# VinAIResearch/Counting-DETR

Hardware: AMD Instinct MI355X
Metric: images/sec FSCD-147 2nd-stage train step (higher is better)
Workload: dtype forward bf16x3 (fp32 operands split hi+lo, 3 bf16 MFMAs per product); data / weight gradients bf16 (both operands rounded to bf16, 1 MFMA per product); fp32 accumulate, fp32 storage, fp32 attention softmax / norms / losses / optimizer; 1 GPU; FSCD-147 2nd-stage train step (ResNet-50-DC5 + RCDA enc6/dec6, Q=300 learned, 800x800, T=[37, 120]), fwd+matcher+loss+bwd+clip+AdamW; images_per_gpu=2, global_batch=2, parallelism=dp1, graph=True, precision=bf16x3, precision_backward=bf16, frozen_stage_prefetch=True

## Files before the change

### counting_detr_amd/csrc/api.hip

```cpp
#include <stdarg.h>
#include <stdio.h>

#include "../../include/cdetr_hip.h"
#include "common.h"

static thread_local char g_err[512] = "";

void cdetr_set_error(const char* fmt, ...) {
    va_list ap;
    va_start(ap, fmt);
    vsnprintf(g_err, sizeof(g_err), fmt, ap);
    va_end(ap);
}

extern "C" const char* cdetr_last_error(void) { return g_err; }
extern "C" int cdetr_abi_version(void) { return CDETR_ABI_VERSION; }

#include <stdlib.h>
#include <string.h>
extern char** environ;
namespace {
struct TuneEnvCheck {
    TuneEnvCheck() {
        if (getenv("CDETR_TUNING") != nullptr || environ == nullptr) return;
        static const char* const knobs[] = {"CDETR_DIRECT_MAX_BLOCKS", "CDETR_GEMM_DL", "CDETR_GEMM_FEWROW_SPLIT", "CDETR_GEMM_SPLITK", "CDETR_GEMM_VARIANT",
                                            "CDETR_LN_BWD_ROWS", "CDETR_LSAP_GENERIC", "CDETR_RCDA_HS", "CDETR_RCDA_PROBE", "CDETR_WGRAD_KP",
                                            "CDETR_WGRAD_VARIANT"};
        for (const char* k : knobs)
            if (getenv(k) != nullptr)
                fprintf(stderr, "libcdetr_hip: %s is set but CDETR_TUNING is not -- per-call tuning knobs are ignored without it\n", k);
    }
} g_tune_env_check;
}
```

### counting_detr_amd/csrc/rcda.hip

```cpp
#include "../../include/cdetr_hip.h"
#include "common.h"
#include <algorithm>
#include <type_traits>
#include <stdlib.h>

namespace {

__device__ __forceinline__ void xcd_slab(int& bx, int& by) {
    const int gx = gridDim.x, total = gx * gridDim.y;
    if (total & 7) return;
    const int lin = by * gx + bx;
    const int l2 = (lin & 7) * (total >> 3) + (lin >> 3);
    by = l2 / gx;
    bx = l2 - by * gx;
}


constexpr int D = 32;
constexpr int QW = 32;

__device__ __forceinline__ float4 ld4(const float* p) { return *reinterpret_cast<const float4*>(p); }

struct FwdSmem {
    int sw, sh;
// ... 204 lines not shown
                                 : make_float4(0.f, 0.f, 0.f, 0.f);

    const float* vbase = d.v + (long)n * H * W * E + head * D;
    constexpr int VSLOTS = (NF * 256 + NT - 1) / NT;
    float4 rv[VSLOTS];
    auto vfetch = [&](int w) {
#pragma unroll
        for (int s = 0; s < VSLOTS; ++s) {
            const int idx = tid + NT * s;
            const int h = idx >> 3, c4 = idx & 7;
            rv[s] = (h < H) ? ld4(vbase + ((long)h * W + w) * E + c4 * 4) : make_float4(0.f, 0.f, 0.f, 0.f);
        }
    };
    auto vstash = [&](int buf) {
#pragma unroll
        for (int s = 0; s < VSLOTS; ++s) {
            const int idx = tid + NT * s;
            const int h = idx >> 3, c4 = idx & 7;
            if (h < H) *reinterpret_cast<float4*>(Vs + buf * Hp * D + h * D + c4 * 4) = rv[s];
        }
    };
    f32x16 acc;
#pragma unroll
    for (int r = 0; r < 16; ++r) acc[r] = 0.f;
    vfetch(0);
    vstash(0);
    __syncthreads();
    for (int w = 0; w < W; ++w) {
        const int buf = w & 1;
        if (w + 1 < W) vfetch(w + 1);
        const float arow = Srow[i32 * sm.sw + w];
        const float* vb = Vs + buf * Hp * D + (g * 4) * D + i32;
        if (PREC == 0) {
#pragma unroll
            for (int kk = 0; kk < KH8; ++kk) {
                if (kk * 8 < Hp) {
                    const float p0 = acol[kk].x * arow, p1 = acol[kk].y * arow, p2 = acol[kk].z * arow, p3 = acol[kk].w * arow;
                    const float b0 = vb[(kk * 8 + 0) * D], b1 = vb[(kk * 8 + 1) * D], b2 = vb[(kk * 8 + 2) * D],
                                b3 = vb[(kk * 8 + 3) * D];
                    acc = __builtin_amdgcn_mfma_f32_32x32x2f32(p0, b0, acc, 0, 0, 0);
                    acc = __builtin_amdgcn_mfma_f32_32x32x2f32(p1, b1, acc, 0, 0, 0);
                    acc = __builtin_amdgcn_mfma_f32_32x32x2f32(p2, b2, acc, 0, 0, 0);
                    acc = __builtin_amdgcn_mfma_f32_32x32x2f32(p3, b3, acc, 0, 0, 0);
                }
            }
        } else {
#pragma unroll
            for (int kp = 0; kp < KH8 / 2; ++kp) {
                if (kp * 16 < Hp) {
                    const int k0 = 2 * kp, k1 = 2 * kp + 1;
                    const bool has1 = k1 * 8 < Hp;
                    const float pa[8] = {acol[k0].x * arow, acol[k0].y * arow, acol[k0].z * arow, acol[k0].w * arow,
                                         acol[k1].x * arow, acol[k1].y * arow, acol[k1].z * arow, acol[k1].w * arow};
                    float vv[8];
#pragma unroll
                    for (int t = 0; t < 4; ++t) {
                        vv[t] = vb[(k0 * 8 + t) * D];
                        vv[4 + t] = has1 ? vb[(k1 * 8 + t) * D] : 0.f;
                    }
                    bf16x8 ah, al, bh, bl;
                    split_bf16x8(pa, ah, al);
                    split_bf16x8(vv, bh, bl);
                    acc = mfma_bf16x3(ah, al, bh, bl, acc);
                }
            }
        }
        if (w + 1 < W) vstash(buf ^ 1);
        __syncthreads();
    }
    mfma_drain(acc);
#pragma unroll
    for (int r = 0; r < 16; ++r) {
        const int qq = qbase + (r & 3) + 8 * (r >> 2) + 4 * g;
        if (qq < L) d.out[((long)n * L + qq) * E + head * D + i32] = acc[r];
    }
}

constexpr int RCDA_WS_COUNTERS = 4096;
constexpr int KSTR = 36;

template <int NT, int TW, int TH, bool PROBE = false>
__device__ __forceinline__ void rcda_scores_mfma(const cdetr_rcda_fwd_desc& d, const FwdSmem& sm, float* smem, float* Srow, float* Scol,
                                                 int tid, int lane, int i32, int g, int n, int head, int qbase, int q, bool qvalid,
                                                 bool save = true, unsigned long long* stamps = nullptr) {
    auto stamp = [&](int i) __attribute__((always_inline)) {
        if constexpr (PROBE) { stamps[i] = __builtin_amdgcn_s_memtime(); asm volatile("s_waitcnt lgkmcnt(0)" ::: "memory"); }
    };
    const int H = d.H, W = d.W, L = d.L, E = d.nh * D;
    const int Wp = (W + 3) & ~3, Hp = (H + 7) & ~7;
    float* Krow = smem + sm.off_k;
    float* Kcol = Krow + W * KSTR;
    {
        const int nk8 = (W + H) * 8;
        for (int base = 0; base < nk8; base += 4 * NT) {
            float4 t[4];
#pragma unroll
            for (int u = 0; u < 4; ++u) {
                const int idx = min(base + tid + NT * u, nk8 - 1);
                const int key = idx >> 3, c4 = idx & 7;
                const float* src = (key < W) ? d.k_row + ((long)n * W + key) * E + head * D + c4 * 4
                                             : d.k_col + ((long)n * H + (key - W)) * E + head * D + c4 * 4;
                t[u] = ld4(src);
            }
#pragma unroll
            for (int u = 0; u < 4; ++u) {
                const int idx = base + tid + NT * u;
                if (idx < nk8) *reinterpret_cast<float4*>(Krow + (idx >> 3) * KSTR + (idx & 7) * 4) = t[u];
            }
        }
    }
    bf16x8 qh[2][2], ql[2][2];
#pragma unroll
    for (int side = 0; side < 2; ++side) {
        const float* qp = (side == 0 ? d.q_row : d.q_col) + ((long)n * L + (qvalid ? q : 0)) * E + head * D + 8 * g;
#pragma unroll
        for (int st = 0; st < 2; ++st) {
            float4 t0 = ld4(qp + 16 * st), t1 = ld4(qp + 16 * st + 4);
            if (!qvalid) { t0 = make_float4(0.f, 0.f, 0.f, 0.f); t1 = t0; }
            const float x[8] = {t0.x, t0.y, t0.z, t0.w, t1.x, t1.y, t1.z, t1.w};
            split_bf16x8(x, qh[side][st], ql[side][st]);
        }
    }
    unsigned long long mrow[2] = {0ull, 0ull}, mcol[2] = {0ull, 0ull};
    if (d.mask_row) {
        const uint8_t* mr = d.mask_row + (long)n * W;
        const uint8_t* mc = d.mask_col + (long)n * H;
        mrow[0] = __ballot(lane < W && mr[min(lane, W - 1)] != 0);
        mcol[0] = __ballot(lane < H && mc[min(lane, H - 1)] != 0);
        if (TW > 2) mrow[1] = __ballot(lane + 64 < W && mr[min(lane + 64, W - 1)] != 0);
        if (TH > 2) mcol[1] = __ballot(lane + 64 < H && mc[min(lane + 64, H - 1)] != 0);
    }
    if constexpr (PROBE) { asm volatile("s_waitcnt vmcnt(0)" ::: "memory"); }
    stamp(0);
    __syncthreads();
    stamp(1);

#pragma unroll
    for (int side = 0; side < 2; ++side) {
        constexpr int TMAX = TW > TH ? TW : TH;
        const int nt = side == 0 ? TW : TH;
        const int nkeys = side == 0 ? W : H, npad = side == 0 ? Wp : Hp;
        const float* Ks = side == 0 ? Krow : Kcol;
        const unsigned long long* mbits = side == 0 ? mrow : mcol;
        float* S = side == 0 ? Srow + i32 * sm.sw : Scol + i32 * sm.sh;
        float sv[TMAX][16];
        float mx = -INFINITY;
#pragma unroll
        for (int t = 0; t < TMAX; ++t) {
            if (t >= nt) break;
            const int kc = min(32 * t + i32, nkeys - 1);
            f32x16 acc = {0.f, 0.f, 0.f, 0.f, 0.f, 0.f, 0.f, 0.f, 0.f, 0.f, 0.f, 0.f, 0.f, 0.f, 0.f, 0.f};
#pragma unroll
            for (int st = 0; st < 2; ++st) {
                const float4 t0 = *reinterpret_cast<const float4*>(Ks + kc * KSTR + 16 * st + 8 * g);
                const float4 t1 = *reinterpret_cast<const float4*>(Ks + kc * KSTR + 16 * st + 8 * g + 4);
                const float x[8] = {t0.x, t0.y, t0.z, t0.w, t1.x, t1.y, t1.z, t1.w};
                bf16x8 ah, al;
                split_bf16x8(x, ah, al);
                acc = mfma_bf16x3(ah, al, qh[side][st], ql[side][st], acc);
            }
            mfma_drain(acc);
            const unsigned chunk = (unsigned)(mbits[t >> 1] >> (32 * (t & 1)));
            const int lim = nkeys - 32 * t - 4 * g;
            const unsigned dead = (chunk >> (4 * g)) | (lim >= 32 ? 0u : (lim <= 0 ? 0xffffffffu : (0xffffffffu << lim)));
#pragma unroll
            for (int r = 0; r < 16; ++r) {
                constexpr unsigned one = 1u;
                const unsigned bit = one << ((r & 3) + 8 * (r >> 2));
                const float v = (dead & bit) ? -INFINITY : acc[r] * d.scale;
                sv[t][r] = v;
                mx = fmaxf(mx, v);
            }
        }
        mx = xhalf_max(mx);
        float sum = 0.f;
#pragma unroll
        for (int t = 0; t < TMAX; ++t) {
            if (t >= nt) break;
#pragma unroll
            for (int r = 0; r < 16; ++r) {
                const float e = __expf(sv[t][r] - mx);
                sv[t][r] = e;
                sum += e;
            }
        }
        sum = xhalf_sum(sum);
        const float inv = 1.f / sum;
#pragma unroll
        for (int t = 0; t < TMAX; ++t) {
            if (t >= nt) break;
#pragma unroll
            for (int r = 0; r < 16; ++r) {
                const int key = 32 * t + (r & 3) + 8 * (r >> 2) + 4 * g;
                S[min(key, npad)] = sv[t][r] * inv;
            }
        }
        stamp(2 + side);
    }
    __syncthreads();
    stamp(4);

    {
        const int nq = min(QW, L - qbase);
        if (nq > 0 && save && d.a_row != nullptr) {
            save_rows(Srow, sm.sw, d.a_row + (((long)n * d.nh + head) * L + qbase) * Wp, nq, Wp, lane);
            save_rows(Scol, sm.sh, d.a_col + (((long)n * d.nh + head) * L + qbase) * Hp, nq, Hp, lane);
        }
    }
    stamp(5);
}

struct Fwd2Smem { int off_v, vts, total; };
__host__ __device__ inline Fwd2Smem fwd2_smem(const FwdSmem& sm, int H, int W, int KS) {
    Fwd2Smem s;
    s.off_v = sm.off_k;
    s.vts = 32 * KS + 8;
    const int vfloats = 2 * 32 * s.vts / 2;
    const int kfloats = (W + H) * KSTR;
    s.total = sm.off_k + (kfloats > vfloats ? kfloats : vfloats);
    return s;
}

template <int NW, int KS, int TH = 2, bool PROBE = false>
__global__ __launch_bounds__(64 * NW) void rcda_fwd2_kernel(const cdetr_rcda_fwd_desc d) {
    unsigned long long pt[5] = {0, 0, 0, 0, 0}, pacc[3] = {0, 0, 0};
    auto now = [&]() __attribute__((always_inline)) -> unsigned long long {
        if constexpr (PROBE) { const unsigned long long t = __builtin_amdgcn_s_memtime(); asm volatile("s_waitcnt lgkmcnt(0)" ::: "memory"); return t; }
        return 0ull;
    };
    pt[0] = now();
    constexpr int NT = 64 * NW, QB = QW * NW;
    constexpr int PD = 4;
    constexpr int NBLK = 16 * 4 * KS;
    constexpr int VB = (NBLK + NT - 1) / NT;
    constexpr int VTS = 32 * KS + 8;
    extern __shared__ __attribute__((aligned(16))) float smem[];
    const int H = d.H, W = d.W, L = d.L, E = d.nh * D;
    const FwdSmem sm = fwd_smem(H, W, NW);
    const int tid = threadIdx.x, lane = tid & 63, wid = tid >> 6;
    const int i32 = lane & 31, g = lane >> 5;
    int bx_ = blockIdx.x, by_ = blockIdx.y;
    xcd_slab(bx_, by_);
    const int n = by_ / d.nh, head = by_ % d.nh;
    const int qbase = bx_ * QB + wid * QW;
    const int q = qbase + i32;
    const bool qvalid = q < L;
    float* Srow = smem + sm.off_srow + wid * QW * sm.sw;
    float* Scol = smem + sm.off_scol + wid * QW * sm.sh;
    const int hs = gridDim.z, hz = blockIdx.z;
    const int hper = (H + hs - 1) / hs;
    const int hb = hz * hper, he = min(H, hb + hper);
    __bf16* VT = reinterpret_cast<__bf16*>(smem + sm.off_k);
    const float* vsrc[VB];
    long vrow[VB][4];
    int vdst[VB];
#pragma unroll
    for (int b = 0; b < VB; ++b) {
        const int blk = tid + NT * b;
        const int wg = (blk < NBLK) ? (blk >> 4) : 0, cp = blk & 15;
        vdst[b] = (blk < NBLK) ? (2 * cp) * VTS + 4 * wg : -1;
        vsrc[b] = d.v + ((long)n * H + min(hb, H - 1)) * W * E + head * D + 2 * cp;
#pragma unroll
        for (int kk = 0; kk < 4; ++kk) vrow[b][kk] = (long)min(4 * wg + kk, W - 1) * E;
    }
    float rv[PD][VB][8];
    const long tileE = (long)W * E;
    int hf = min(hb, H - 1);
    auto vfetch = [&](float (&r)[VB][8]) __attribute__((always_inline)) {
#pragma unroll
        for (int b = 0; b < VB; ++b) {
#pragma unroll
            for (int kk = 0; kk < 4; ++kk) {
                const float2 t = *reinterpret_cast<const float2*>(vsrc[b] + vrow[b][kk]);
                r[b][2 * kk] = t.x;
                r[b][2 * kk + 1] = t.y;
            }
        }
        ++hf;
        if (hf < H) {
#pragma unroll
            for (int b = 0; b < VB; ++b) vsrc[b] += tileE;
        }
    };
    auto vstash = [&](const float (&r)[VB][8], int buf) __attribute__((always_inline)) {
#pragma unroll
        for (int b = 0; b < VB; ++b) {
            if (vdst[b] < 0) continue;
            __bf16* dst = VT + buf * 32 * VTS + vdst[b];
            stash_split4(dst, 16 * KS, r[b][0], r[b][2], r[b][4], r[b][6]);
            stash_split4(dst + VTS, 16 * KS, r[b][1], r[b][3], r[b][5], r[b][7]);
        }
    };

    unsigned long long sst[6] = {0, 0, 0, 0, 0, 0};
    if (H <= 32 * TH) rcda_scores_mfma<NT, (KS + 1) / 2, TH, PROBE>(d, sm, smem, Srow, Scol, tid, lane, i32, g, n, head, qbase, q, qvalid, hz == 0, sst);
    else rcda_scores<NT>(d, sm, smem, Srow, Scol, tid, lane, i32, g, n, head, qbase, q, qvalid);
    pt[1] = now();

    bf16x8 bh[KS], bl[KS];
#pragma unroll
    for (int s = 0; s < KS; ++s) {
        float x[8];
#pragma unroll
        for (int j = 0; j < 8; ++j) {
            const int w = 16 * s + 8 * g + j;
            x[j] = (w < W) ? Srow[i32 * sm.sw + w] : 0.f;
        }
        split_bf16x8(x, bh[s], bl[s]);
    }

    float outT[16];
#pragma unroll
    for (int r = 0; r < 16; ++r) outT[r] = 0.f;
    const f32x16 zero = {0.f, 0.f, 0.f, 0.f, 0.f, 0.f, 0.f, 0.f, 0.f, 0.f, 0.f, 0.f, 0.f, 0.f, 0.f, 0.f};

    vfetch(rv[0]); vfetch(rv[1]); vfetch(rv[2]); vfetch(rv[3]);
    vstash(rv[0], 0);
    __syncthreads();
    pt[2] = now();
    auto step = [&](auto U, int h) __attribute__((always_inline)) {
        constexpr int u = decltype(U)::value;
        const unsigned long long s0 = now();
        vfetch(rv[u]);
        const unsigned long long s1 = now();
        const float acolh = (h < he) ? Scol[i32 * sm.sh + h] : 0.f;
        const __bf16* vt = VT + (u & 1) * 32 * VTS + i32 * VTS + 8 * g;
        f32x16 T = zero;
#pragma unroll
        for (int s = 0; s < KS; ++s) {
            const bf16x8 ah = *reinterpret_cast<const bf16x8*>(vt + 16 * s);
            const bf16x8 al = *reinterpret_cast<const bf16x8*>(vt + 16 * KS + 16 * s);
            T = mfma_bf16x3(ah, al, bh[s], bl[s], T);
        }
#pragma unroll
        for (int r = 0; r < 16; ++r) outT[r] = fmaf(acolh, T[r], outT[r]);
        unsigned long long s2 = 0;
        if constexpr (PROBE) { asm volatile("" :: "v"(outT[0]), "v"(outT[15])); s2 = now(); }
        vstash(rv[(u + 1) % PD], (u + 1) & 1);
        const unsigned long long s3 = now();
        __syncthreads();
        if constexpr (PROBE) {
            const unsigned long long s4 = now();
            pacc[0] += s4 - s3; pacc[1] += s2 - s1; pacc[2] += (s1 - s0) + (s3 - s2);
        }
    };
    for (int h0 = hb; h0 < he; h0 += PD) {
        step(std::integral_constant<int, 0>{}, h0);
        step(std::integral_constant<int, 1>{}, h0 + 1);
        step(std::integral_constant<int, 2>{}, h0 + 2);
        step(std::integral_constant<int, 3>{}, h0 + 3);
    }
    pt[3] = now();
    if (hs > 1) {
        int* cnt = reinterpret_cast<int*>(d.ws);
        float* wsp = reinterpret_cast<float*>(cnt + RCDA_WS_COUNTERS);
        const int tile = blockIdx.y * gridDim.x + blockIdx.x;
        float* mine = wsp + ((long)tile * hs + hz) * 16 * NT + tid;
#pragma unroll
        for (int r = 0; r < 16; ++r) __hip_atomic_store(mine + r * NT, outT[r], __ATOMIC_RELAXED, __HIP_MEMORY_SCOPE_AGENT);
        __builtin_amdgcn_s_waitcnt(0);
        __syncthreads();
        int* flag = reinterpret_cast<int*>(smem + sm.off_k);
        if (tid == 0) {
            const int old = __hip_atomic_fetch_add(cnt + tile, 1, __ATOMIC_RELAXED, __HIP_MEMORY_SCOPE_AGENT);
            const int last = (old == hs - 1) ? 1 : 0;
            if (last) __hip_atomic_store(cnt + tile, 0, __ATOMIC_RELAXED, __HIP_MEMORY_SCOPE_AGENT);
            *flag = last;
        }
        __syncthreads();
        if (*flag == 0) return;
        float sum[16];
#pragma unroll
        for (int r = 0; r < 16; ++r) sum[r] = 0.f;
        for (int z = 0; z < hs; ++z) {
            if (z == hz) {
#pragma unroll
                for (int r = 0; r < 16; ++r) sum[r] += outT[r];
            } else {
                const float* other = wsp + ((long)tile * hs + z) * 16 * NT + tid;
                float t[16];
#pragma unroll
                for (int r = 0; r < 16; ++r) t[r] = __hip_atomic_load(other + r * NT, __ATOMIC_RELAXED, __HIP_MEMORY_SCOPE_AGENT);
#pragma unroll
                for (int r = 0; r < 16; ++r) sum[r] += t[r];
            }
        }
#pragma unroll
        for (int r = 0; r < 16; ++r) outT[r] = sum[r];
    }
    if (qvalid) {
        float* op = d.out + ((long)n * L + q) * E + head * D + 4 * g;
#pragma unroll
        for (int j = 0; j < 4; ++j)
            *reinterpret_cast<float4*>(op + 8 * j) = make_float4(outT[4 * j], outT[4 * j + 1], outT[4 * j + 2], outT[4 * j + 3]);
    }
    if constexpr (PROBE) {
        asm volatile("s_waitcnt vmcnt(0)" ::: "memory");
        pt[4] = now();
        if (lane == 0) {
            unsigned long long* o = reinterpret_cast<unsigned long long*>(d.ws) + ((long)(blockIdx.y * gridDim.x + blockIdx.x) * NW + wid) * 16;
            o[0] = pt[0]; o[1] = pt[1]; o[2] = pt[2]; o[3] = pt[3]; o[4] = pt[4]; o[5] = pacc[0]; o[6] = pacc[1]; o[7] = pacc[2];
#pragma unroll
            for (int i = 0; i < 6; ++i) o[8 + i] = sst[i];
        }
    }
}

constexpr int BWD_CG = 2;
struct BwdSmem {
    int sw, sh, su, off_u, off_r, off_kk, total;
};
__host__ __device__ inline BwdSmem bwd_smem(int H, int W, int NF, int NW, bool with_k = false) {
    BwdSmem s;
    const int Wp = (W + 3) & ~3, Hp = (H + 7) & ~7;
    s.sw = Wp + 1;
    s.sh = Hp + 1;
    s.su = s.sw > s.sh ? s.sw : s.sh;
    s.off_u = 0;
    int u = NW * QW * s.su;
    const int v = 2 * BWD_CG * (32 * NF) * 36;
    if (v > u) u = v;
    s.off_r = (u + 3) & ~3;
    s.total = s.off_r + NW * QW * s.sw;
    s.off_kk = (s.total + 3) & ~3;
    if (with_k) s.total = s.off_kk + (W + H) * D;
    return s;
}

template <int NF, int NW, int PREC, int TERMS = 3, bool PROBE = false>
__device__ __forceinline__ void rcda_bwd_body(const cdetr_rcda_bwd_desc& d, const int bx, const int by) {
    unsigned long long pst[7] = {0, 0, 0, 0, 0, 0, 0};
    auto stamp = [&](int i) __attribute__((always_inline)) {
        if constexpr (PROBE) { pst[i] = __builtin_amdgcn_s_memtime(); asm volatile("s_waitcnt lgkmcnt(0)" ::: "memory"); }
    };
    auto flush_probe = [&]() __attribute__((always_inline)) {
        if constexpr (PROBE) {
            asm volatile("s_waitcnt vmcnt(0)" ::: "memory");
            if ((threadIdx.x & 63) == 0) {
                unsigned long long* o = reinterpret_cast<unsigned long long*>(d.ds_row) + ((long)(by * gridDim.x + bx) * NW + (threadIdx.x >> 6)) * 16;
#pragma unroll
                for (int i = 0; i < 7; ++i) o[i] = pst[i];
            }
        }
    };
    stamp(0);
    constexpr int NT = 64 * NW, QB = QW * NW;
    extern __shared__ __attribute__((aligned(16))) float smem[];
    constexpr int VS = 36;
    constexpr int HR = 32 * NF;
    const int H = d.H, W = d.W, L = d.L, E = d.nh * D;
    const int Wp = (W + 3) & ~3, Hp = (H + 7) & ~7;
    const BwdSmem sm = bwd_smem(H, W, NF, NW, d.dq_row != nullptr);
    const int tid = threadIdx.x, lane = tid & 63, wid = tid >> 6;
    const int i32 = lane & 31, g = lane >> 5;
    const int n = by / d.nh, head = by % d.nh;
    const int qbase = bx * QB + wid * QW;
    const int q = qbase + i32;
    const bool qvalid = q < L;
    const int nq = min(QW, L - qbase);

    constexpr int KP = 4;
    const int nk8 = (W + H) * 8;
    const bool kpre_ok = d.dq_row != nullptr && nk8 <= KP * NT;
    float4 kpre[KP];
#pragma unroll
    for (int u = 0; u < KP; ++u) kpre[u] = make_float4(0.f, 0.f, 0.f, 0.f);
    if (kpre_ok) {
#pragma unroll
        for (int u = 0; u < KP; ++u) {
            const int idx = min(tid + NT * u, nk8 - 1);
            const int key = idx >> 3, c4 = idx & 7;
            const float* src = (key < W) ? d.k_row + ((long)n * W + key) * E + head * D + c4 * 4
                                         : d.k_col + ((long)n * H + (key - W)) * E + head * D + c4 * 4;
            kpre[u] = ld4(src);
        }
    }

    float* Acol = smem + sm.off_u + wid * QW * sm.su;
    float* Arow = smem + sm.off_r + wid * QW * sm.sw;
    float* dArow = Arow;
    float* Vs = smem + sm.off_u;

    float dob[4][4];
// ... 676 lines not shown
template <int NF, int NW>
int launch_rcda_bwd_all(const cdetr_rcda_bwd_desc& d, hipStream_t st, int hgroups, int slices, int per) {
    const int bytes = std::max(bwd_smem(d.H, d.W, NF, NW, d.dq_row != nullptr).total * 4, dv2_smem().total * 4);
    int rc;
    const int nqb = (d.L + QW * NW - 1) / (QW * NW);
    dim3 grid(nqb + hgroups * slices, d.N * d.nh);
    if (d.precision == 3) {
        if ((rc = set_smem(rcda_bwd_all_kernel<NF, NW, 1>, bytes, "cdetr_rcda_bwd"))) return rc;
        hipLaunchKernelGGL((rcda_bwd_all_kernel<NF, NW, 1>), grid, dim3(512), bytes, st, d, nqb, hgroups, per);
    } else {
        if ((rc = set_smem(rcda_bwd_all_kernel<NF, NW, 3>, bytes, "cdetr_rcda_bwd"))) return rc;
        hipLaunchKernelGGL((rcda_bwd_all_kernel<NF, NW, 3>), grid, dim3(512), bytes, st, d, nqb, hgroups, per);
    }
    return cdetr_launch_status("cdetr_rcda_bwd(dS+dV)");
}
template <int NF, int NW>
int launch_rcda_bwd(const cdetr_rcda_bwd_desc& d, hipStream_t st) {
    const BwdSmem sm = bwd_smem(d.H, d.W, NF, NW, d.dq_row != nullptr);
    const int bytes = sm.total * 4;
    int rc;
    dim3 grid((d.L + QW * NW - 1) / (QW * NW), d.N * d.nh), block(64 * NW);
    if constexpr (NF == 4) {
        if (d.precision == 3) {
            if ((rc = set_smem(rcda_bwd_kernel<NF, NW, 1, 1>, bytes, "cdetr_rcda_bwd"))) return rc;
            hipLaunchKernelGGL((rcda_bwd_kernel<NF, NW, 1, 1>), grid, block, bytes, st, d);
            return cdetr_launch_status("cdetr_rcda_bwd(dS)");
        }
        if (d.precision >= 1) {
            if ((rc = set_smem(rcda_bwd_kernel<NF, NW, 1>, bytes, "cdetr_rcda_bwd"))) return rc;
            hipLaunchKernelGGL((rcda_bwd_kernel<NF, NW, 1>), grid, block, bytes, st, d);
            return cdetr_launch_status("cdetr_rcda_bwd(dS)");
        }
    }
    if ((rc = set_smem(rcda_bwd_kernel<NF, NW, 0>, bytes, "cdetr_rcda_bwd"))) return rc;
    hipLaunchKernelGGL((rcda_bwd_kernel<NF, NW, 0>), grid, block, bytes, st, d);
    return cdetr_launch_status("cdetr_rcda_bwd(dS)");
}
inline bool rcda_wg5(int L, int NH) {
    const long wg4 = (long)((L + QW * 4 - 1) / (QW * 4)) * NH, wg5 = (long)((L + QW * 5 - 1) / (QW * 5)) * NH;
    return wg4 > 256 && wg4 <= 512 && wg5 <= 256;
}
inline int fwd2_slices(const cdetr_rcda_fwd_desc& d, int base, int nt, int lds_bytes) {
    if (!d.ws || base > RCDA_WS_COUNTERS) return 1;
    int hs;
    const char* f = cdetr_tune_env("CDETR_RCDA_HS");
    if (f) hs = atoi(f);
    else {
        const int per_cu = lds_bytes > 0 ? std::max(1, std::min(4, (160 * 1024) / lds_bytes)) : 1;
        (void)per_cu;
        hs = 256 / base;
    }
    hs = std::min(std::min(hs, 8), d.H / 8);
    const long avail = (long)d.ws_bytes - (long)RCDA_WS_COUNTERS * 4;
    while (hs > 1 && (long)base * hs * 16 * nt * 4 > avail) --hs;
    return hs < 1 ? 1 : hs;
}
inline int rcda_probe() {
    const char* p = cdetr_tune_env("CDETR_RCDA_PROBE");
    return p ? atoi(p) : 0;
}

}

extern "C" int cdetr_rcda_fwd(const cdetr_rcda_fwd_desc* dp, void* stream) {
    CDETR_CHECK_ARG(dp != nullptr, "cdetr_rcda_fwd: null descriptor");
    const cdetr_rcda_fwd_desc d = *dp;
    CDETR_CHECK_ARG(d.N > 0 && d.L > 0 && d.H > 0 && d.W > 0 && d.nh > 0, "cdetr_rcda_fwd: bad sizes");
    CDETR_CHECK_ARG(d.H <= 128 && d.W <= 1024, "cdetr_rcda_fwd: H must be <= 128 (got %d)", d.H);
    CDETR_CHECK_ARG(d.q_row && d.q_col && d.k_row && d.k_col && d.v && d.out, "cdetr_rcda_fwd: null pointer");
    CDETR_CHECK_ARG((d.a_row != nullptr) == (d.a_col != nullptr), "cdetr_rcda_fwd: a_row and a_col are saved together or not at all (both NULL: inference)");
    hipStream_t st = reinterpret_cast<hipStream_t>(stream);
    if (d.precision == 1 && d.W <= 96) {
        const int ks = (d.W + 15) / 16;
        auto go = [&](auto kern, int NWv, int KSv = 0, bool sliced = true) -> int {
            const FwdSmem sm = fwd_smem(d.H, d.W, NWv);
            const int bytes = fwd2_smem(sm, d.H, d.W, KSv ? KSv : ks).total * 4;
            int rc;
            if ((rc = set_smem(kern, bytes, "cdetr_rcda_fwd"))) return rc;
            dim3 grid((d.L + QW * NWv - 1) / (QW * NWv), d.N * d.nh), block(64 * NWv);
            if (sliced) grid.z = fwd2_slices(d, (int)(grid.x * grid.y), 64 * NWv, bytes);
            hipLaunchKernelGGL(kern, grid, block, bytes, st, d);
            return cdetr_launch_status("cdetr_rcda_fwd");
        };
        if (const int probe = rcda_probe(); probe && d.ws && ks == 4 && d.H <= 64)
            return probe == 5 ? go(rcda_fwd2_kernel<5, 4, 2, true>, 5, 0, false) : go(rcda_fwd2_kernel<4, 4, 2, true>, 4, 0, false);
        if (ks == 4 && rcda_wg5(d.L, d.N * d.nh)) return go(rcda_fwd2_kernel<5, 4>, 5);
        if (ks > 4 || d.H > 64) {
            if (d.H > 64 && d.H <= 96) return ks <= 4 ? go(rcda_fwd2_kernel<4, 4, 3>, 4, 4) : go(rcda_fwd2_kernel<4, 6, 3>, 4, 6);
            if (ks <= 4) return go(rcda_fwd2_kernel<4, 4>, 4, 4);
            return ks == 5 ? go(rcda_fwd2_kernel<4, 5>, 4) : go(rcda_fwd2_kernel<4, 6>, 4);
        }
        if (ks == 1) return go(rcda_fwd2_kernel<4, 1>, 4);
        if (ks == 2) return go(rcda_fwd2_kernel<4, 2>, 4);
        if (ks == 3) return go(rcda_fwd2_kernel<4, 3>, 4);
        return go(rcda_fwd2_kernel<4, 4>, 4);
    }
    if (d.H <= 32) return launch_rcda_fwd<1>(d, st);
    if (d.H <= 64) return launch_rcda_fwd<2>(d, st);
    return launch_rcda_fwd<4>(d, st);
}

extern "C" int cdetr_rcda_bwd(const cdetr_rcda_bwd_desc* dp, void* stream) {
    CDETR_CHECK_ARG(dp != nullptr, "cdetr_rcda_bwd: null descriptor");
    const cdetr_rcda_bwd_desc d = *dp;
    CDETR_CHECK_ARG(d.N > 0 && d.L > 0 && d.H > 0 && d.W > 0 && d.nh > 0, "cdetr_rcda_bwd: bad sizes");
    CDETR_CHECK_ARG(d.H <= 128 && d.W <= 1024, "cdetr_rcda_bwd: H must be <= 128 (got %d)", d.H);
    CDETR_CHECK_ARG(d.d_out && d.a_row && d.a_col && d.v && d.d_v, "cdetr_rcda_bwd: null pointer");
    CDETR_CHECK_ARG((d.ds_row && d.ds_col) || (!d.ds_row && !d.ds_col && d.dk_row),
                    "cdetr_rcda_bwd: ds_row / ds_col may only be omitted (both) when the fused q / k gradients are requested");
    CDETR_CHECK_ARG(!d.dq_row || (d.dq_col && d.k_row && d.k_col), "cdetr_rcda_bwd: dq_row needs dq_col, k_row and k_col");
    CDETR_CHECK_ARG(!d.dk_row || (d.dq_row && d.dk_col && d.q_row && d.q_col && d.precision >= 1),
                    "cdetr_rcda_bwd: dk_row needs dk_col, q_row, q_col, the dq_* outputs and a split-bf16 precision (1 or 3)");
    hipStream_t st = reinterpret_cast<hipStream_t>(stream);
    const int NF = d.H <= 32 ? 1 : (d.H <= 64 ? 2 : 4);
    const int Wp = (d.W + 3) & ~3;
    int rc;
    if (const int probe = rcda_probe(); probe && NF == 2 && d.precision == 3 && d.ds_row && d.dk_row) {
        const int NWp = probe == 5 ? 5 : 4;
        const BwdSmem sm = bwd_smem(d.H, d.W, 2, NWp, true);
        dim3 grid((d.L + QW * NWp - 1) / (QW * NWp), d.N * d.nh), block(64 * NWp);
        if (NWp == 5) {
            if ((rc = set_smem(rcda_bwd_kernel<2, 5, 1, 1, true>, sm.total * 4, "cdetr_rcda_bwd"))) return rc;
            hipLaunchKernelGGL((rcda_bwd_kernel<2, 5, 1, 1, true>), grid, block, sm.total * 4, st, d);
        } else {
            if ((rc = set_smem(rcda_bwd_kernel<2, 4, 1, 1, true>, sm.total * 4, "cdetr_rcda_bwd"))) return rc;
            hipLaunchKernelGGL((rcda_bwd_kernel<2, 4, 1, 1, true>), grid, block, sm.total * 4, st, d);
        }
        return cdetr_launch_status("cdetr_rcda_bwd(probe)");
    }
    const bool wg5 = NF == 2 && rcda_wg5(d.L, d.N * d.nh);
    const bool dv2 = d.precision >= 1;
    if (dv2) {
        const int hgroups = ((d.H + 7) / 8) * ((Wp + 63) / 64);
        const long base = (long)hgroups * d.N * d.nh;
        const long ds_wgs = (long)((d.L + QW * 4 - 1) / (QW * 4)) * d.N * d.nh;
        const int dv2_target = ds_wgs <= 128 ? 112 : 224;
        int slices = (int)((dv2_target + base - 1) / base);
        const int max_slices = (d.L + 255) / 256;
        if (slices > max_slices) slices = max_slices;
        if (slices < 1) slices = 1;
        int per = (d.L + slices - 1) / slices;
        per = ((per + 63) / 64) * 64;
        slices = (d.L + per - 1) / per;
        if (NF == 1) return launch_rcda_bwd_all<1, 4>(d, st, hgroups, slices, per);
        if (NF == 2) return wg5 ? launch_rcda_bwd_all<2, 5>(d, st, hgroups, slices, per) : launch_rcda_bwd_all<2, 4>(d, st, hgroups, slices, per);
        if ((rc = launch_rcda_bwd<4, 4>(d, st))) return rc;
        const int bytes = dv2_smem().total * 4;
        if (d.precision == 3) {
            if ((rc = set_smem(rcda_dv2_kernel<1>, bytes, "cdetr_rcda_bwd(dV)"))) return rc;
            hipLaunchKernelGGL(rcda_dv2_kernel<1>, dim3(hgroups, d.N * d.nh, slices), dim3(512), bytes, st, d, per);
        } else {
            if ((rc = set_smem(rcda_dv2_kernel<3>, bytes, "cdetr_rcda_bwd(dV)"))) return rc;
            hipLaunchKernelGGL(rcda_dv2_kernel<3>, dim3(hgroups, d.N * d.nh, slices), dim3(512), bytes, st, d, per);
        }
        return cdetr_launch_status("cdetr_rcda_bwd(dV)");
    }
    if (NF == 1) rc = launch_rcda_bwd<1, 4>(d, st);
    else if (NF == 2) rc = wg5 ? launch_rcda_bwd<2, 5>(d, st) : launch_rcda_bwd<2, 4>(d, st);
    else rc = launch_rcda_bwd<4, 4>(d, st);
    if (rc) return rc;
    const int bytes = (64 * 32 * NF + 64 * Wp + 64 * 32) * 4;
    const int wgroups = (d.W + 3) / 4;
    const long base = (long)wgroups * d.N * d.nh;
    int slices = (int)((1024 + base - 1) / base);
    const int max_slices = (d.L + 127) / 128;
    if (slices > max_slices) slices = max_slices;
    if (slices < 1) slices = 1;
    int per = (d.L + slices - 1) / slices;
    per = ((per + 63) / 64) * 64;
    slices = (d.L + per - 1) / per;
    dim3 grid(wgroups, d.N * d.nh, slices), block(256);
    auto dv = [&](auto kern) -> int {
        if ((rc = set_smem(kern, bytes, "cdetr_rcda_bwd(dV)"))) return rc;
        hipLaunchKernelGGL(kern, grid, block, bytes, st, d, per);
        return cdetr_launch_status("cdetr_rcda_bwd(dV)");
    };
    if (NF == 1) return dv(rcda_dv_kernel<1, 0>);
    if (NF == 2) return dv(rcda_dv_kernel<2, 0>);
// ... 3 lines not shown
```

Baseline: 246.9 images/s.

## Split RCDA forward across paired wave groups for row/column scores and alternating H

Adds a paired-group RCDA forward kernel that doubles the threads per block. One half computes the row-side scores and the other the column-side scores. Both halves then walk alternating H rows of the value pass with their own double-buffered staging, and their partial outputs are combined through shared memory. The aim is to cut per-wave serial latency in the score and value loops. In exchange the block uses more shared memory and registers and adds a cross-half reduction. The split-H global reduction is factored into a shared helper.

```diff
diff --git a/counting_detr_amd/csrc/api.hip b/counting_detr_amd/csrc/api.hip
--- a/counting_detr_amd/csrc/api.hip
+++ b/counting_detr_amd/csrc/api.hip
@@ -24,7 +24,7 @@
     TuneEnvCheck() {
         if (getenv("CDETR_TUNING") != nullptr || environ == nullptr) return;
         static const char* const knobs[] = {"CDETR_DIRECT_MAX_BLOCKS", "CDETR_GEMM_DL", "CDETR_GEMM_FEWROW_SPLIT", "CDETR_GEMM_SPLITK", "CDETR_GEMM_VARIANT",
-                                            "CDETR_LN_BWD_ROWS", "CDETR_LSAP_GENERIC", "CDETR_RCDA_HS", "CDETR_RCDA_PROBE", "CDETR_WGRAD_KP",
+                                            "CDETR_LN_BWD_ROWS", "CDETR_LSAP_GENERIC", "CDETR_RCDA_HS", "CDETR_RCDA_NG", "CDETR_RCDA_PROBE", "CDETR_WGRAD_KP",
                                             "CDETR_WGRAD_VARIANT"};
         for (const char* k : knobs)
             if (getenv(k) != nullptr)
diff --git a/counting_detr_amd/csrc/rcda.hip b/counting_detr_amd/csrc/rcda.hip
--- a/counting_detr_amd/csrc/rcda.hip
+++ b/counting_detr_amd/csrc/rcda.hip
@@ -310,7 +310,7 @@
 template <int NT, int TW, int TH, bool PROBE = false>
 __device__ __forceinline__ void rcda_scores_mfma(const cdetr_rcda_fwd_desc& d, const FwdSmem& sm, float* smem, float* Srow, float* Scol,
                                                  int tid, int lane, int i32, int g, int n, int head, int qbase, int q, bool qvalid,
-                                                 bool save = true, unsigned long long* stamps = nullptr) {
+                                                 bool save = true, unsigned long long* stamps = nullptr, int sides = 3) {
     auto stamp = [&](int i) __attribute__((always_inline)) {
         if constexpr (PROBE) { stamps[i] = __builtin_amdgcn_s_memtime(); asm volatile("s_waitcnt lgkmcnt(0)" ::: "memory"); }
     };
@@ -340,6 +340,7 @@
     bf16x8 qh[2][2], ql[2][2];
 #pragma unroll
     for (int side = 0; side < 2; ++side) {
+        if (!((sides >> side) & 1)) continue;
         const float* qp = (side == 0 ? d.q_row : d.q_col) + ((long)n * L + (qvalid ? q : 0)) * E + head * D + 8 * g;
 #pragma unroll
         for (int st = 0; st < 2; ++st) {
@@ -365,6 +366,7 @@
 
 #pragma unroll
     for (int side = 0; side < 2; ++side) {
+        if (!((sides >> side) & 1)) { stamp(2 + side); continue; }
         constexpr int TMAX = TW > TH ? TW : TH;
         const int nt = side == 0 ? TW : TH;
         const int nkeys = side == 0 ? W : H, npad = side == 0 ? Wp : Hp;
@@ -431,32 +433,78 @@
     {
         const int nq = min(QW, L - qbase);
         if (nq > 0 && save && d.a_row != nullptr) {
-            save_rows(Srow, sm.sw, d.a_row + (((long)n * d.nh + head) * L + qbase) * Wp, nq, Wp, lane);
-            save_rows(Scol, sm.sh, d.a_col + (((long)n * d.nh + head) * L + qbase) * Hp, nq, Hp, lane);
+            if (sides & 1) save_rows(Srow, sm.sw, d.a_row + (((long)n * d.nh + head) * L + qbase) * Wp, nq, Wp, lane);
+            if (sides & 2) save_rows(Scol, sm.sh, d.a_col + (((long)n * d.nh + head) * L + qbase) * Hp, nq, Hp, lane);
         }
     }
     stamp(5);
 }
 
 struct Fwd2Smem { int off_v, vts, total; };
-__host__ __device__ inline Fwd2Smem fwd2_smem(const FwdSmem& sm, int H, int W, int KS) {
+__host__ __device__ inline Fwd2Smem fwd2_smem(const FwdSmem& sm, int H, int W, int KS, int pair_groups = 0) {
     Fwd2Smem s;
     s.off_v = sm.off_k;
     s.vts = 32 * KS + 8;
-    const int vfloats = 2 * 32 * s.vts / 2;
+    const int vfloats = (pair_groups ? 4 : 2) * 32 * s.vts / 2;
     const int kfloats = (W + H) * KSTR;
-    s.total = sm.off_k + (kfloats > vfloats ? kfloats : vfloats);
+    const int xfloats = pair_groups * 16 * 64;
+    const int m = kfloats > vfloats ? kfloats : vfloats;
+    s.total = sm.off_k + (m > xfloats ? m : xfloats);
     return s;
 }
 
-template <int NW, int KS, int TH = 2, bool PROBE = false>
+template <int NTQ>
+__device__ __forceinline__ void rcda_fwd2_finish(const cdetr_rcda_fwd_desc& d, int* flag, float (&outT)[16], bool owner, int tq,
+                                                 int n, int head, int q, bool qvalid, int g) {
+    const int hs = gridDim.z, hz = blockIdx.z;
+    if (hs > 1) {
+        int* cnt = reinterpret_cast<int*>(d.ws);
+        float* wsp = reinterpret_cast<float*>(cnt + RCDA_WS_COUNTERS);
+        const int tile = blockIdx.y * gridDim.x + blockIdx.x;
+        if (owner) {
+            float* mine = wsp + ((long)tile * hs + hz) * 16 * NTQ + tq;
+#pragma unroll
+            for (int r = 0; r < 16; ++r) __hip_atomic_store(mine + r * NTQ, outT[r], __ATOMIC_RELAXED, __HIP_MEMORY_SCOPE_AGENT);
+        }
+        __builtin_amdgcn_s_waitcnt(0);
+        __syncthreads();
+        if (threadIdx.x == 0) {
+            const int old = __hip_atomic_fetch_add(cnt + tile, 1, __ATOMIC_RELAXED, __HIP_MEMORY_SCOPE_AGENT);
+            const int last = (old == hs - 1) ? 1 : 0;
+            if (last) __hip_atomic_store(cnt + tile, 0, __ATOMIC_RELAXED, __HIP_MEMORY_SCOPE_AGENT);
+            *flag = last;
+        }
+        __syncthreads();
+        if (*flag == 0 || !owner) return;
+        float sum[16];
+#pragma unroll
+        for (int r = 0; r < 16; ++r) sum[r] = 0.f;
+        for (int z = 0; z < hs; ++z) {
+            if (z == hz) {
+#pragma unroll
+                for (int r = 0; r < 16; ++r) sum[r] += outT[r];
+            } else {
+                const float* other = wsp + ((long)tile * hs + z) * 16 * NTQ + tq;
+                float t[16];
+#pragma unroll
+                for (int r = 0; r < 16; ++r) t[r] = __hip_atomic_load(other + r * NTQ, __ATOMIC_RELAXED, __HIP_MEMORY_SCOPE_AGENT);
+#pragma unroll
+                for (int r = 0; r < 16; ++r) sum[r] += t[r];
+            }
+        }
+#pragma unroll
+        for (int r = 0; r < 16; ++r) outT[r] = sum[r];
+    }
+    if (owner && qvalid) {
+        float* op = d.out + ((long)n * d.L + q) * (d.nh * D) + head * D + 4 * g;
+#pragma unroll
+        for (int j = 0; j < 4; ++j)
+            *reinterpret_cast<float4*>(op + 8 * j) = make_float4(outT[4 * j], outT[4 * j + 1], outT[4 * j + 2], outT[4 * j + 3]);
+    }
+}
+
+template <int NW, int KS, int TH = 2>
 __global__ __launch_bounds__(64 * NW) void rcda_fwd2_kernel(const cdetr_rcda_fwd_desc d) {
-    unsigned long long pt[5] = {0, 0, 0, 0, 0}, pacc[3] = {0, 0, 0};
-    auto now = [&]() __attribute__((always_inline)) -> unsigned long long {
-        if constexpr (PROBE) { const unsigned long long t = __builtin_amdgcn_s_memtime(); asm volatile("s_waitcnt lgkmcnt(0)" ::: "memory"); return t; }
-        return 0ull;
-    };
-    pt[0] = now();
     constexpr int NT = 64 * NW, QB = QW * NW;
     constexpr int PD = 4;
     constexpr int NBLK = 16 * 4 * KS;
@@ -520,10 +568,8 @@
         }
     };
 
-    unsigned long long sst[6] = {0, 0, 0, 0, 0, 0};
-    if (H <= 32 * TH) rcda_scores_mfma<NT, (KS + 1) / 2, TH, PROBE>(d, sm, smem, Srow, Scol, tid, lane, i32, g, n, head, qbase, q, qvalid, hz == 0, sst);
+    if (H <= 32 * TH) rcda_scores_mfma<NT, (KS + 1) / 2, TH>(d, sm, smem, Srow, Scol, tid, lane, i32, g, n, head, qbase, q, qvalid, hz == 0);
     else rcda_scores<NT>(d, sm, smem, Srow, Scol, tid, lane, i32, g, n, head, qbase, q, qvalid);
-    pt[1] = now();
 
     bf16x8 bh[KS], bl[KS];
 #pragma unroll
@@ -545,14 +591,125 @@
     vfetch(rv[0]); vfetch(rv[1]); vfetch(rv[2]); vfetch(rv[3]);
     vstash(rv[0], 0);
     __syncthreads();
-    pt[2] = now();
     auto step = [&](auto U, int h) __attribute__((always_inline)) {
         constexpr int u = decltype(U)::value;
+        vfetch(rv[u]);
+        const float acolh = (h < he) ? Scol[i32 * sm.sh + h] : 0.f;
+        const __bf16* vt = VT + (u & 1) * 32 * VTS + i32 * VTS + 8 * g;
+        f32x16 T = zero;
+#pragma unroll
+        for (int s = 0; s < KS; ++s) {
+            const bf16x8 ah = *reinterpret_cast<const bf16x8*>(vt + 16 * s);
+            const bf16x8 al = *reinterpret_cast<const bf16x8*>(vt + 16 * KS + 16 * s);
+            T = mfma_bf16x3(ah, al, bh[s], bl[s], T);
+        }
+#pragma unroll
+        for (int r = 0; r < 16; ++r) outT[r] = fmaf(acolh, T[r], outT[r]);
+        vstash(rv[(u + 1) % PD], (u + 1) & 1);
+        __syncthreads();
+    };
+    for (int h0 = hb; h0 < he; h0 += PD) {
+        step(std::integral_constant<int, 0>{}, h0);
+        step(std::integral_constant<int, 1>{}, h0 + 1);
+        step(std::integral_constant<int, 2>{}, h0 + 2);
+        step(std::integral_constant<int, 3>{}, h0 + 3);
+    }
+    rcda_fwd2_finish<NT>(d, reinterpret_cast<int*>(smem + sm.off_k), outT, true, tid, n, head, q, qvalid, g);
+}
+
+template <int NG, int KS, bool PROBE = false>
+__global__ __launch_bounds__(128 * NG) void rcda_fwd2p_kernel(const cdetr_rcda_fwd_desc d) {
+    unsigned long long pt[5] = {0, 0, 0, 0, 0}, pacc[3] = {0, 0, 0};
+    auto now = [&]() __attribute__((always_inline)) -> unsigned long long {
+        if constexpr (PROBE) { const unsigned long long t = __builtin_amdgcn_s_memtime(); asm volatile("s_waitcnt lgkmcnt(0)" ::: "memory"); return t; }
+        return 0ull;
+    };
+    pt[0] = now();
+    constexpr int NT = 128 * NG, NTQ = 64 * NG, QB = QW * NG;
+    constexpr int PD = 3;
+    constexpr int NBLK = 16 * 4 * KS;
+    constexpr int VTS = 32 * KS + 8;
+    static_assert(KS <= 4 && 2 * NBLK <= NT, "one staging block per thread: the two live tiles are 128 KS blocks");
+    extern __shared__ __attribute__((aligned(16))) float smem[];
+    const int H = d.H, W = d.W, L = d.L, E = d.nh * D;
+    const FwdSmem sm = fwd_smem(H, W, NG);
+    const int tid = threadIdx.x, lane = tid & 63, wid = __builtin_amdgcn_readfirstlane(tid >> 6);
+    const int half = wid >= NG ? 1 : 0, grp = wid - half * NG;
+    const int i32 = lane & 31, g = lane >> 5;
+    int bx_ = blockIdx.x, by_ = blockIdx.y;
+    xcd_slab(bx_, by_);
+    const int n = by_ / d.nh, head = by_ % d.nh;
+    const int qbase = bx_ * QB + grp * QW;
+    const int q = qbase + i32;
+    const bool qvalid = q < L;
+    float* Srow = smem + sm.off_srow + grp * QW * sm.sw;
+    float* Scol = smem + sm.off_scol + grp * QW * sm.sh;
+    const int hs = gridDim.z, hz = blockIdx.z;
+    const int hper = (H + hs - 1) / hs;
+    const int hb = hz * hper, he = min(H, hb + hper);
+    __bf16* VT = reinterpret_cast<__bf16*>(smem + sm.off_k);
+    const int tp = (tid >= NBLK) ? 1 : 0;
+    const int blk = tid - tp * NBLK;
+    const bool stager = tid < 2 * NBLK;
+    const int swg = stager ? (blk >> 4) : 0, scp = blk & 15;
+    const int vdst = stager ? tp * 2 * 32 * VTS + (2 * scp) * VTS + 4 * swg : -1;
+    int hf = min(hb + tp, H - 1);
+    const float* vsrc = d.v + ((long)n * H + hf) * W * E + head * D + 2 * scp;
+    int vrow[4];
+#pragma unroll
+    for (int kk = 0; kk < 4; ++kk) vrow[kk] = min(4 * swg + kk, W - 1) * E;
+    float rv[PD][8];
+    const long tileE = (long)W * E;
+    auto vfetch = [&](float (&r)[8]) __attribute__((always_inline)) {
+#pragma unroll
+        for (int kk = 0; kk < 4; ++kk) {
+            const float2 t = *reinterpret_cast<const float2*>(vsrc + vrow[kk]);
+            r[2 * kk] = t.x;
+            r[2 * kk + 1] = t.y;
+        }
+        const int adv = min(2, H - 1 - hf);
+        hf += adv;
+        vsrc += adv == 2 ? 2 * tileE : (adv == 1 ? tileE : 0);
+    };
+    auto vstash = [&](const float (&r)[8], int buf) __attribute__((always_inline)) {
+        if (vdst < 0) return;
+        __bf16* dst = VT + buf * 32 * VTS + vdst;
+        stash_split4(dst, 16 * KS, r[0], r[2], r[4], r[6]);
+        stash_split4(dst + VTS, 16 * KS, r[1], r[3], r[5], r[7]);
+    };
+
+    vfetch(rv[0]); vfetch(rv[1]); vfetch(rv[2]);
+    unsigned long long sst[6] = {0, 0, 0, 0, 0, 0};
+    rcda_scores_mfma<NT, (KS + 1) / 2, 2, PROBE>(d, sm, smem, Srow, Scol, tid, lane, i32, g, n, head, qbase, q, qvalid, hz == 0, sst, 1 << half);
+    pt[1] = now();
+
+    bf16x8 bh[KS], bl[KS];
+#pragma unroll
+    for (int s = 0; s < KS; ++s) {
+        float x[8];
+#pragma unroll
+        for (int j = 0; j < 8; ++j) {
+            const int w = 16 * s + 8 * g + j;
+            x[j] = (w < W) ? Srow[i32 * sm.sw + w] : 0.f;
+        }
+        split_bf16x8(x, bh[s], bl[s]);
+    }
+
+    float outT[16];
+#pragma unroll
+    for (int r = 0; r < 16; ++r) outT[r] = 0.f;
+    const f32x16 zero = {0.f, 0.f, 0.f, 0.f, 0.f, 0.f, 0.f, 0.f, 0.f, 0.f, 0.f, 0.f, 0.f, 0.f, 0.f, 0.f};
+
+    vstash(rv[0], 0);
+    __syncthreads();
+    pt[2] = now();
+    auto step = [&](auto U, auto B, int h) __attribute__((always_inline)) {
+        constexpr int u = decltype(U)::value, b = decltype(B)::value;
         const unsigned long long s0 = now();
         vfetch(rv[u]);
         const unsigned long long s1 = now();
         const float acolh = (h < he) ? Scol[i32 * sm.sh + h] : 0.f;
-        const __bf16* vt = VT + (u & 1) * 32 * VTS + i32 * VTS + 8 * g;
+        const __bf16* vt = VT + (2 * half + b) * 32 * VTS + i32 * VTS + 8 * g;
         f32x16 T = zero;
 #pragma unroll
         for (int s = 0; s < KS; ++s) {
@@ -564,7 +721,7 @@
         for (int r = 0; r < 16; ++r) outT[r] = fmaf(acolh, T[r], outT[r]);
         unsigned long long s2 = 0;
         if constexpr (PROBE) { asm volatile("" :: "v"(outT[0]), "v"(outT[15])); s2 = now(); }
-        vstash(rv[(u + 1) % PD], (u + 1) & 1);
+        vstash(rv[(u + 1) % PD], b ^ 1);
         const unsigned long long s3 = now();
         __syncthreads();
         if constexpr (PROBE) {
@@ -572,61 +729,32 @@
             pacc[0] += s4 - s3; pacc[1] += s2 - s1; pacc[2] += (s1 - s0) + (s3 - s2);
         }
     };
-    for (int h0 = hb; h0 < he; h0 += PD) {
-        step(std::integral_constant<int, 0>{}, h0);
-        step(std::integral_constant<int, 1>{}, h0 + 1);
-        step(std::integral_constant<int, 2>{}, h0 + 2);
-        step(std::integral_constant<int, 3>{}, h0 + 3);
+    using I0 = std::integral_constant<int, 0>; using I1 = std::integral_constant<int, 1>; using I2 = std::integral_constant<int, 2>;
+    for (int h = hb + half, hend = he + half;;) {
+        step(I0{}, I0{}, h); if ((h += 2) >= hend) break;
+        step(I1{}, I1{}, h); if ((h += 2) >= hend) break;
+        step(I2{}, I0{}, h); if ((h += 2) >= hend) break;
+        step(I0{}, I1{}, h); if ((h += 2) >= hend) break;
+        step(I1{}, I0{}, h); if ((h += 2) >= hend) break;
+        step(I2{}, I1{}, h); if ((h += 2) >= hend) break;
     }
     pt[3] = now();
-    if (hs > 1) {
-        int* cnt = reinterpret_cast<int*>(d.ws);
-        float* wsp = reinterpret_cast<float*>(cnt + RCDA_WS_COUNTERS);
-        const int tile = blockIdx.y * gridDim.x + blockIdx.x;
-        float* mine = wsp + ((long)tile * hs + hz) * 16 * NT + tid;
-#pragma unroll
-        for (int r = 0; r < 16; ++r) __hip_atomic_store(mine + r * NT, outT[r], __ATOMIC_RELAXED, __HIP_MEMORY_SCOPE_AGENT);
-        __builtin_amdgcn_s_waitcnt(0);
-        __syncthreads();
-        int* flag = reinterpret_cast<int*>(smem + sm.off_k);
-        if (tid == 0) {
-            const int old = __hip_atomic_fetch_add(cnt + tile, 1, __ATOMIC_RELAXED, __HIP_MEMORY_SCOPE_AGENT);
-            const int last = (old == hs - 1) ? 1 : 0;
-            if (last) __hip_atomic_store(cnt + tile, 0, __ATOMIC_RELAXED, __HIP_MEMORY_SCOPE_AGENT);
-            *flag = last;
-        }
-        __syncthreads();
-        if (*flag == 0) return;
-        float sum[16];
-#pragma unroll
-        for (int r = 0; r < 16; ++r) sum[r] = 0.f;
-        for (int z = 0; z < hs; ++z) {
-            if (z == hz) {
-#pragma unroll
-                for (int r = 0; r < 16; ++r) sum[r] += outT[r];
-            } else {
-                const float* other = wsp + ((long)tile * hs + z) * 16 * NT + tid;
-                float t[16];
-#pragma unroll
-                for (int r = 0; r < 16; ++r) t[r] = __hip_atomic_load(other + r * NT, __ATOMIC_RELAXED, __HIP_MEMORY_SCOPE_AGENT);
-#pragma unroll
-                for (int r = 0; r < 16; ++r) sum[r] += t[r];
-            }
-        }
-#pragma unroll
-        for (int r = 0; r < 16; ++r) outT[r] = sum[r];
-    }
-    if (qvalid) {
-        float* op = d.out + ((long)n * L + q) * E + head * D + 4 * g;
-#pragma unroll
-        for (int j = 0; j < 4; ++j)
-            *reinterpret_cast<float4*>(op + 8 * j) = make_float4(outT[4 * j], outT[4 * j + 1], outT[4 * j + 2], outT[4 * j + 3]);
-    }
+    float* xch = smem + sm.off_k + grp * 16 * 64 + lane;
+    if (half) {
+#pragma unroll
+        for (int r = 0; r < 16; ++r) xch[64 * r] = outT[r];
+    }
+    __syncthreads();
+    if (!half) {
+#pragma unroll
+        for (int r = 0; r < 16; ++r) outT[r] += xch[64 * r];
+    }
+    rcda_fwd2_finish<NTQ>(d, reinterpret_cast<int*>(smem + sm.off_k), outT, half == 0, tid, n, head, q, qvalid, g);
     if constexpr (PROBE) {
         asm volatile("s_waitcnt vmcnt(0)" ::: "memory");
         pt[4] = now();
         if (lane == 0) {
-            unsigned long long* o = reinterpret_cast<unsigned long long*>(d.ws) + ((long)(blockIdx.y * gridDim.x + blockIdx.x) * NW + wid) * 16;
+            unsigned long long* o = reinterpret_cast<unsigned long long*>(d.ws) + ((long)(blockIdx.y * gridDim.x + blockIdx.x) * 2 * NG + wid) * 16;
             o[0] = pt[0]; o[1] = pt[1]; o[2] = pt[2]; o[3] = pt[3]; o[4] = pt[4]; o[5] = pacc[0]; o[6] = pacc[1]; o[7] = pacc[2];
 #pragma unroll
             for (int i = 0; i < 6; ++i) o[8 + i] = sst[i];
@@ -1469,18 +1597,31 @@
             hipLaunchKernelGGL(kern, grid, block, bytes, st, d);
             return cdetr_launch_status("cdetr_rcda_fwd");
         };
+        auto pair = [&](auto kern, int NGv, bool sliced = true) -> int {
+            const FwdSmem sm = fwd_smem(d.H, d.W, NGv);
+            const int bytes = fwd2_smem(sm, d.H, d.W, ks, NGv).total * 4;
+            int rc;
+            if ((rc = set_smem(kern, bytes, "cdetr_rcda_fwd"))) return rc;
+            dim3 grid((d.L + QW * NGv - 1) / (QW * NGv), d.N * d.nh), block(128 * NGv);
+            if (sliced) grid.z = fwd2_slices(d, (int)(grid.x * grid.y), 64 * NGv, bytes);
+            hipLaunchKernelGGL(kern, grid, block, bytes, st, d);
+            return cdetr_launch_status("cdetr_rcda_fwd");
+        };
         if (const int probe = rcda_probe(); probe && d.ws && ks == 4 && d.H <= 64)
-            return probe == 5 ? go(rcda_fwd2_kernel<5, 4, 2, true>, 5, 0, false) : go(rcda_fwd2_kernel<4, 4, 2, true>, 4, 0, false);
-        if (ks == 4 && rcda_wg5(d.L, d.N * d.nh)) return go(rcda_fwd2_kernel<5, 4>, 5);
+            return probe == 5 ? pair(rcda_fwd2p_kernel<5, 4, true>, 5, false) : pair(rcda_fwd2p_kernel<4, 4, true>, 4, false);
         if (ks > 4 || d.H > 64) {
+            if (ks == 4 && rcda_wg5(d.L, d.N * d.nh)) return go(rcda_fwd2_kernel<5, 4>, 5);
             if (d.H > 64 && d.H <= 96) return ks <= 4 ? go(rcda_fwd2_kernel<4, 4, 3>, 4, 4) : go(rcda_fwd2_kernel<4, 6, 3>, 4, 6);
             if (ks <= 4) return go(rcda_fwd2_kernel<4, 4>, 4, 4);
             return ks == 5 ? go(rcda_fwd2_kernel<4, 5>, 4) : go(rcda_fwd2_kernel<4, 6>, 4);
         }
-        if (ks == 1) return go(rcda_fwd2_kernel<4, 1>, 4);
-        if (ks == 2) return go(rcda_fwd2_kernel<4, 2>, 4);
-        if (ks == 3) return go(rcda_fwd2_kernel<4, 3>, 4);
-        return go(rcda_fwd2_kernel<4, 4>, 4);
+        bool wg5 = ks == 4 && rcda_wg5(d.L, d.N * d.nh);
+        if (const char* f = cdetr_tune_env("CDETR_RCDA_NG"); f && ks == 4) wg5 = atoi(f) == 5;
+        if (wg5) return pair(rcda_fwd2p_kernel<5, 4>, 5);
+        if (ks == 1) return pair(rcda_fwd2p_kernel<4, 1>, 4);
+        if (ks == 2) return pair(rcda_fwd2p_kernel<4, 2>, 4);
+        if (ks == 3) return pair(rcda_fwd2p_kernel<4, 3>, 4);
+        return pair(rcda_fwd2p_kernel<4, 4>, 4);
     }
     if (d.H <= 32) return launch_rcda_fwd<1>(d, st);
     if (d.H <= 64) return launch_rcda_fwd<2>(d, st);
```

Result: no change. 248.9 images/s, median of 6 (+0.8%).
